# peterropac/Aegolius

Measured on AMD Instinct MI355X. Metric: Mpoints/sec SDF eval, 1024^3 grid, 10-prim smooth-union tree, higher is better.
Workload: dtype f32

## Files before the change

aegolius_amd/csrc/sdfk_codegen.cpp:

```cpp
#include "sdfk_codegen.h"

#include <algorithm>
#include <cstdio>
#include <cstring>
#include <map>
#include <set>

#include "sdfk_embedded.inc"

std::string sdfk_vector_prelude() { return std::string(kEmbeddedDevice) + "\n" + kEmbeddedVecdev + "\n"; }

static const char kWrappers[] = R"SDFKW(
template <int VEC, typename SRC>
static __device__ __forceinline__ void sdfk_body(const float* __restrict__ PRM, const float* __restrict__ TAB,
                                                 const SRC& src, long long off, long long n,
                                                 float* __restrict__ out, const float* __restrict__ aux,
                                                 long long aux_stride, unsigned* __restrict__ flags, unsigned thr) {
    const long long block_base = (long long)sdfk_bx() * (SDFK_BLOCK * VEC);
    const unsigned lane_off = sdfk_tx() * VEC;
#ifdef SDFK_FLAGS                                              // the flag-writing build of this flavour (its own code object:
    {                                                          // carried as a run-time branch it cost the field kernels registers)
        const bool active = block_base + lane_off < n;
        unsigned nib = 0u;
        if (active) {
// ... 737 lines not shown
        if (__builtin_bit_cast(unsigned, x0) != __builtin_bit_cast(unsigned, meta->xy[b][SDFK_RROWS - 1].x)) {
            int s = 1;
            while (s < SDFK_RROWS - 1 && __builtin_bit_cast(unsigned, meta->xy[b][s].x) == __builtin_bit_cast(unsigned, x0)) ++s;
            r0 = sb / NZP ? s : 0;
            r1 = sb / NZP ? SDFK_RROWS : s;
        }
    }
    const float2 pa = meta->xy[b][r0], pe = meta->xy[b][r1 - 1];
    const float za = meta->z[b][r0 * SDFK_RZ + i0], ze = meta->z[b][(r1 - 1) * SDFK_RZ + i0 + ZPS - 1];
    const float cx = 0.5f * (pa.x + pe.x), cy = 0.5f * (pa.y + pe.y), cz = 0.5f * (za + ze);
    float r2 = 0.0f;
#pragma unroll 1
    for (int rr = r0; rr < r1; ++rr) {
        const int r = rr - r0;
        const float2 p = meta->xy[b][r0 + r];
        const float dx = p.x - cx, dy = p.y - cy;
        float zm = 0.0f;
#pragma unroll
        for (int i = 0; i < ZPS; i += 4) {
            const float4 q = *reinterpret_cast<const float4*>(&meta->z[b][(r0 + r) * SDFK_RZ + i0 + i]);
            zm = sd_rawmax(sd_rawmax(zm, sd_abs(q.x - cz)), sd_rawmax(sd_abs(q.y - cz), sd_rawmax(sd_abs(q.z - cz), sd_abs(q.w - cz))));
        }
        r2 = sd_rawmax(r2, sd_fma(zm, zm, sd_fma(dx, dx, dy * dy)));
    }
    const float rho = 1.00001f * sqrtf(r2) + 1e-30f;
#ifdef SDFK_FLAT
    return make_float4(cx, cz, cy, rho);                         // (the staged coordinate is y, xy holds (x, z = 0))
#else
    return make_float4(cx, cy, cz, rho);
#endif
}
#endif

#if defined(SDFK_CHAIN) && !defined(SDFK_CELLS)
// Chain mode, one WAVE per brick: which children run on this brick, from the leaf values at its centre. A hard min (max:
// signs flipped, e_k = +-d_k) is exact, associative and commutative, so the ORDER of the chain does not matter for a
// decision: child k can be dropped wherever some other child j stays below it on the whole brick, and with j = the child
// that is smallest at the centre that is guaranteed by e_k - m >= thr, m = min_j e_j, thr = K rho + margins with
// K = the largest Lipschitz sum of the chain (any pair). No prefix minimum, no "restart" level: one reduction for m, then
// 64 children per step — compare, ballot, and the survivors written as a LIST in index order, so that the evaluation
// never looks at a child it skips and still combines the others in the chain's order. (Tighter than the sequential rule,
// which compares a child with its predecessors only.)
static __device__ __forceinline__ void sdfk_chain_fold(sdfk_rowmeta* meta, int b, int lane) {
    const float4 cc = meta->bound[b];
    const float rho = cc.w, cmag = 1e-6f * (fabsf(cc.x) + fabsf(cc.y) + fabsf(cc.z) + rho);
    constexpr int NW = (SDFK_NLEAF + 63) / 64;
    float m = 3.0e38f;
#pragma unroll 4
    for (int j = 0; j < NW; ++j) {
        const int k = 64 * j + lane;
        if (k < SDFK_NLEAF) m = fminf(m, SDFK_CHAIN_SGN * meta->leafval[k * SDFK_NCEN + b]);
    }
#pragma unroll
    for (int o = 1; o < 64; o <<= 1) m = fminf(m, __shfl_xor(m, o));
    const float thr0 = 1.0001f * SDFK_CHAIN_KMAX * rho + SDFK_CHAIN_KMAX * cmag + 1e-6f * (1.0f + fabsf(m));
    int n_out = 0;
#pragma unroll 1
    for (int j = 0; j < NW; ++j) {
        const int k = 64 * j + lane;
        const bool in = k < SDFK_NLEAF;
        const float e = in ? SDFK_CHAIN_SGN * meta->leafval[k * SDFK_NCEN + b] : 3.0e38f;
        const bool run = in && !(e - m >= thr0 + 1e-6f * fabsf(e));
        const unsigned long long bits = __ballot(run);
        if (run) meta->alist[b][n_out + __builtin_popcountll(bits & ((1ull << lane) - 1ull))] = (unsigned short)k;
        n_out += __builtin_popcountll(bits);
    }
    if (lane == 0) meta->nalive[b] = (unsigned)n_out;
}
#endif

#ifdef SDFK_CELLS
// rows of row block rb plus the cell of brick (rb, window c) and that cell's sphere (wave-uniform; scalar loads)
static __device__ __forceinline__ void sdfk_brick_cell(const sdfk_rowgeom& g, const sdfk_cells& cl, unsigned rb, unsigned c,
                                                       long long& r0, long long& rend, uint2& span, float4& S) {
    unsigned slot, blk;
    sdfk_block_rows(g, rb, r0, rend, &slot, &blk);
    const unsigned sx = slot == 0xffffffffu ? 0u : cl.lv.xoff + slot;
    const unsigned cell = ((sx >> cl.lv.lx) * cl.lv.ncy + (blk >> cl.lv.ly)) * cl.lv.ncz + (c >> cl.lv.lz);
    S = make_float4(0.0f, 0.0f, 0.0f, -1.0f);
    span = make_uint2(0u, SDFK_ALL_ALIVE);
    // (the launch is padded with bricks beyond the last one: their row block does not exist, and neither does a cell for it)
    if (cl.enabled && r0 < rend && cell < cl.ncells) {
        const uint2 sp = cl.span[cell];
        span = make_uint2(__builtin_amdgcn_readfirstlane(sp.x), __builtin_amdgcn_readfirstlane(sp.y));
        const float4 t = cl.sph[cell];
#ifdef SDFK_FLAT
        S = make_float4(t.x, t.z, t.y, t.w);                   // (the registers of phase A hold (x, z, y))
#else
        S = t;
#endif
    }
}
#endif
#if defined(SDFK_CHAIN) && defined(SDFK_CELLS)
// The same decision from the CELL's candidate list: one member per lane, evaluated at the brick's centre on the spot (no
// table of leaf values in LDS) — the first 64 stay in a register, longer lists are evaluated a second time for the
// comparison. A brick that is not inside its cell's sphere, or whose cell has no list, takes every member.
// `sp` (the cell's span) and `first` (this lane's entry of the first batch) were loaded BEFORE the coordinates were waited
// for, so the only memory round trip left between the bounds and the decision is the members' parameters.
static __device__ __forceinline__ void sdfk_chain_fold_cells(sdfk_rowmeta* meta, int b, int lane, const sdfk_cells& cl, uint2 sp,
                                                             unsigned first, const float* __restrict__ PRM,
                                                             const float* __restrict__ TAB) {
    const float4 cc = meta->bound[b];
    const V3T<float> ctr = {cc.x, cc.y, cc.z};
    const float rho = cc.w, cmag = 1e-6f * (fabsf(cc.x) + fabsf(cc.y) + fabsf(cc.z) + rho);
    unsigned off = 0u, cnt = SDFK_NLEAF;
    bool listed = false;
    if (cl.enabled && __builtin_amdgcn_readfirstlane(meta->inside[b]) != 0u && sp.y != SDFK_ALL_ALIVE) {
        off = sp.x; cnt = sp.y; listed = true;
    }
    float m = 3.0e38f, e0 = 3.0e38f;
    unsigned r0 = 0u;
#pragma unroll 1
    for (unsigned j0 = 0u; j0 < cnt; j0 += 64u) {
        const unsigned j = j0 + (unsigned)lane;
        const bool in = j < cnt;
        unsigned rec = 0u;
        if (in) rec = listed ? (j0 == 0u ? first : cl.cand[off + j]) : sdfk_member_record(j);
        float e = 3.0e38f;
        if (in) e = SDFK_CHAIN_SGN * sdfk_leaf_rec<float>(rec, ctr, PRM, TAB);
        if (j0 == 0u) { e0 = e; r0 = rec; }
        m = fminf(m, e);
    }
#pragma unroll
    for (int o = 1; o < 64; o <<= 1) m = fminf(m, __shfl_xor(m, o));
    const float thr0 = 1.0001f * SDFK_CHAIN_KMAX * rho + SDFK_CHAIN_KMAX * cmag + 1e-6f * (1.0f + fabsf(m));
    unsigned n_out = 0u;
#pragma unroll 1
    for (unsigned j0 = 0u; j0 < cnt; j0 += 64u) {
        const unsigned j = j0 + (unsigned)lane;
        const bool in = j < cnt;
        unsigned rec = r0;
        float e = e0;
        if (j0 != 0u) {
            rec = in ? (listed ? cl.cand[off + j] : sdfk_member_record(j)) : 0u;
            e = 3.0e38f;
            if (in) e = SDFK_CHAIN_SGN * sdfk_leaf_rec<float>(rec, ctr, PRM, TAB);
        }
        const bool run = in && !(e - m >= thr0 + 1e-6f * fabsf(e));
        const unsigned long long bits = __ballot(run);
        const unsigned pos = n_out + (unsigned)__builtin_popcountll(bits & ((1ull << lane) - 1ull));
        if (run && pos < SDFK_ALIST_CAP) meta->alist[b][pos] = rec;
        n_out += (unsigned)__builtin_popcountll(bits);
    }
    // more survivors than the list in LDS holds (dense scenes): the brick runs its cell's whole candidate list straight from
    // memory — a superset in the chain's order — and every member only where there is no such list
    if (lane == 0) {
        meta->nalive[b] = n_out <= SDFK_ALIST_CAP ? n_out : (listed ? SDFK_LIST_ALIVE : SDFK_ALL_ALIVE);
        meta->aspan[b] = make_uint2(off, cnt);
    }
}
#endif

// phases A and B of the tile of this workgroup; returns this wave's first brick (row block, window)
#ifdef SDFK_CELLS
#define SDFK_CELLS_PARAM , const sdfk_cells& cl
#define SDFK_CELLS_PASS , cl
#else
#define SDFK_CELLS_PARAM
#define SDFK_CELLS_PASS
#endif
template <typename SRC>
static __device__ __forceinline__ void sdfk_rows_prepare(const float* __restrict__ PRM, const float* __restrict__ TAB,
                                                         const SRC& s, const sdfk_rowgeom& g, sdfk_rowmeta* meta,
                                                         unsigned tile, unsigned& rb0, unsigned& c0 SDFK_CELLS_PARAM) {
    const int lane = sdfk_tx() & 63, wave = __builtin_amdgcn_readfirstlane(sdfk_tx() >> 6);
    const unsigned q0 = tile * SDFK_RNBRICK + wave * SDFK_RWBRICKS;            // first brick of this wave
    rb0 = sdfk_udiv(q0, g.nchunk, g.inv_nchunk);                // (back in an SGPR: what is derived from it stays scalar)
    c0 = q0 - rb0 * g.nchunk;
    unsigned rb = rb0, c = c0;
#if SDFK_RWBRICKS <= 2 && !defined(SDFK_NOHOIST)
    // two-wave workgroups on the north-star grid; with four bricks per wave the registers this takes cost more)
    sdfk_rowregs hregs[SDFK_RWBRICKS];
    bool live[SDFK_RWBRICKS];
#ifdef SDFK_CELLS
    uint2 cspan[SDFK_RWBRICKS];
    unsigned cfirst[SDFK_RWBRICKS];
    float4 csph[SDFK_RWBRICKS];
#endif
#pragma unroll
    for (int j = 0; j < SDFK_RWBRICKS; ++j) {
        long long r0, rend;
#ifdef SDFK_CELLS
        sdfk_brick_cell(g, cl, rb, c, r0, rend, cspan[j], csph[j]);
        cfirst[j] = 0u;                                          // the lane's entry of the list's first batch: in flight with the coordinates
        if (cspan[j].y != SDFK_ALL_ALIVE && (unsigned)lane < cspan[j].y) cfirst[j] = cl.cand[cspan[j].x + (unsigned)lane];
#else
        sdfk_block_rows(g, rb, r0, rend);
#endif
        live[j] = q0 + j < g.nbricks && r0 < rend;               // (blocks of the last plane beyond the slab: nothing)
        if (live[j]) sdfk_rows_load(s, g, r0, rend, c, lane, hregs[j]);
        if (++c == g.nchunk) { c = 0; ++rb; }
    }
#pragma unroll
    for (int j = 0; j < SDFK_RWBRICKS; ++j)
#ifdef SDFK_CELLS
        if (live[j]) sdfk_rows_bounds(hregs[j], lane, meta, wave * SDFK_RWBRICKS + j, csph[j]);
#else
        if (live[j]) sdfk_rows_bounds(hregs[j], lane, meta, wave * SDFK_RWBRICKS + j);
#endif
        else if (lane == 0) { meta->bound[wave * SDFK_RWBRICKS + j] = make_float4(0.0f, 0.0f, 0.0f, 1.0f); meta->uniform[wave * SDFK_RWBRICKS + j] = 0u; }   // (masks: never read)
#else
#ifdef SDFK_CELLS
    bool live[SDFK_RWBRICKS];
    uint2 cspan[SDFK_RWBRICKS];
    unsigned cfirst[SDFK_RWBRICKS];
#endif
#pragma unroll
    for (int j = 0; j < SDFK_RWBRICKS; ++j) {
        long long r0, rend;
#ifdef SDFK_CELLS
        float4 csph;
        sdfk_brick_cell(g, cl, rb, c, r0, rend, cspan[j], csph);
        cfirst[j] = 0u;
        if (cspan[j].y != SDFK_ALL_ALIVE && (unsigned)lane < cspan[j].y) cfirst[j] = cl.cand[cspan[j].x + (unsigned)lane];
        live[j] = q0 + j < g.nbricks && r0 < rend;
#else
        sdfk_block_rows(g, rb, r0, rend);
#endif
#ifdef SDFK_ABLATE_EDGE
        if (q0 + j < g.nbricks && r0 < rend && sdfk_interior(g.L, c)) {
#else
        if (q0 + j < g.nbricks && r0 < rend) {
#endif
            sdfk_rowregs regs;
            sdfk_rows_load(s, g, r0, rend, c, lane, regs);
#ifdef SDFK_CELLS
            sdfk_rows_bounds(regs, lane, meta, wave * SDFK_RWBRICKS + j, csph);
#else
            sdfk_rows_bounds(regs, lane, meta, wave * SDFK_RWBRICKS + j);
#endif
        } else if (lane == 0) {                                   // a dead brick still meets a probe lane: harmless values
            meta->bound[wave * SDFK_RWBRICKS + j] = make_float4(0.0f, 0.0f, 0.0f, 1.0f);
            meta->uniform[wave * SDFK_RWBRICKS + j] = 0u;
        }
        if (++c == g.nchunk) { c = 0; ++rb; }
    }
#endif
    __syncthreads();
#if defined(SDFK_CHAIN) && defined(SDFK_CELLS)
    // every wave folds ITS bricks from their cells' lists: nothing crosses waves any more (no probe centres, no table of
    // leaf values, two barriers fewer than the path below)
#pragma unroll
    for (int j = 0; j < SDFK_RWBRICKS; ++j) {
        const int b = wave * SDFK_RWBRICKS + j;
#ifdef SDFK_ABLATE_PROBE
        if (lane == 0) { meta->alist[b][0] = sdfk_member_record(0u); meta->nalive[b] = live[j] ? 1u : 0u; }
#else
        if (live[j]) sdfk_chain_fold_cells(meta, b, lane, cl, cspan[j], cfirst[j], PRM, TAB);
        else if (lane == 0) meta->nalive[b] = 0u;
#endif
    }
    __syncthreads();
    return;
#endif
#if defined(SDFK_SIMT) && !defined(SDFK_CELLS)
    // lane-parallel probe: probe centres -> every leaf at every centre (all lanes) -> one fold lane per centre ANDs its
    // skip decisions into the brick's mask (a subtree is skipped only if every sub-brick allows it)
    if (sdfk_tx() < SDFK_NCEN) {
        const unsigned b = sdfk_tx() / SDFK_NSUB, sb = sdfk_tx() % SDFK_NSUB;
        float4 cc = meta->bound[b];
#if SDFK_NSUB > 1
        if (meta->uniform[b]) cc = sdfk_sub_centre(meta, b, sb);
#else
        (void)sb;
#endif
        meta->cen[sdfk_tx()] = cc;
    }
    __syncthreads();
#ifndef SDFK_ABLATE_PROBE
    sdfk_probe_leaves(meta->cen, meta->leafval, PRM, TAB);
    __syncthreads();
#ifdef SDFK_CHAIN
#pragma unroll 1
    for (int j = 0; j < SDFK_RWBRICKS; ++j)
        if (q0 + j < g.nbricks) sdfk_chain_fold(meta, wave * SDFK_RWBRICKS + j, lane);
    __syncthreads();
    return;
#else
    if (sdfk_tx() < SDFK_NCEN && tile * SDFK_RNBRICK + sdfk_tx() / SDFK_NSUB < g.nbricks) {
        const float4 cc = meta->cen[sdfk_tx()];
        V3T<float> ctr = {cc.x, cc.y, cc.z};
        unsigned long long mk[SDFK_NMASK];
        sdfk_probe_fold(meta->leafval, sdfk_tx(), ctr, cc.w, PRM, mk);
#pragma unroll
        for (int w = 0; w < SDFK_NMASK; ++w)
            __hip_atomic_fetch_and(&meta->mask[w][sdfk_tx() / SDFK_NSUB], mk[w], __ATOMIC_RELAXED, __HIP_MEMORY_SCOPE_WORKGROUP);
    }
#endif
#else
    if (sdfk_tx() < SDFK_RNBRICK) {
#pragma unroll
        for (int w = 0; w < SDFK_NMASK; ++w) meta->mask[w][sdfk_tx()] = 0ull;
    }
#endif
    __syncthreads();
    return;
#endif
    if (sdfk_tx() < SDFK_RNBRICK && tile * SDFK_RNBRICK + sdfk_tx() < g.nbricks) {
        const float4 bb = meta->bound[sdfk_tx()];
        V3T<float> ctr = {bb.x, bb.y, bb.z};
        unsigned long long mk[SDFK_NMASK];
#pragma unroll
        for (int w = 0; w < SDFK_NMASK; ++w) mk[w] = 0ull;
#if !defined(SDFK_ABLATE_PROBE) && !defined(SDFK_CHAIN)
        sdfk_probe_r(ctr, bb.w, PRM, TAB, mk);
#endif
#pragma unroll
        for (int w = 0; w < SDFK_NMASK; ++w) meta->mask[w][sdfk_tx()] = mk[w];
    }
    __syncthreads();
}

template <typename SRC>
static __device__ __forceinline__ void sdfk_rows_kernel(const float* __restrict__ PRM, const float* __restrict__ TAB,
                                                        const SRC& s, const sdfk_rowgeom& g, float* __restrict__ out,
                                                        unsigned* __restrict__ flags, unsigned thr SDFK_CELLS_PARAM) {
    __shared__ __attribute__((aligned(16))) sdfk_rowmeta meta;
#ifdef SDFK_LDSPAD
    if (g.L == 0xffffffffu) meta.pad[sdfk_tx()] = 1.0f;
#endif
    const int lane = sdfk_tx() & 63, wave = __builtin_amdgcn_readfirstlane(sdfk_tx() >> 6);
    const int lr = lane / SDFK_RLPR;
    const int zq = (lane % SDFK_RLPR) * (2 * SDFK_NP);
#ifndef SDFK_RTILES
#define SDFK_RTILES 1
#endif
#ifndef SDFK_XGROUP
#ifdef SDFK_FLAT                         // flat grids (rows of 16385 points: 513 windows): short runs — the 50-member union at
#define SDFK_XGROUP 4
#else
#define SDFK_XGROUP (SDFK_RNBRICK <= 4 ? 16 : (SDFK_RNBRICK <= 8 ? 8 : 4))    // runs of about 64 bricks: two row blocks at 1025
#endif
#endif
#pragma unroll 1
  for (unsigned tt = 0; tt < SDFK_RTILES; ++tt) {
    // Workgroups go round-robin to the 8 XCDs: an XCD takes runs of SDFK_XGROUP consecutive tiles (the grid is a
    // multiple of 8 * SDFK_XGROUP) instead of every eighth tile, while all XCDs stay in the same neighbourhood of the
    // in all of them (DESIGN 9.1).
    const unsigned xg_t = sdfk_bx() / 8;
    const unsigned tile = (((xg_t / SDFK_XGROUP) * 8 + sdfk_bx() % 8) * SDFK_XGROUP + xg_t % SDFK_XGROUP) * SDFK_RTILES + tt;
    if (tile * SDFK_RNBRICK >= g.nbricks) break;
    if (tt) __syncthreads();
    unsigned rb, c;
    sdfk_rows_prepare(PRM, TAB, s, g, &meta, tile, rb, c SDFK_CELLS_PASS);
    const unsigned q0 = tile * SDFK_RNBRICK + wave * SDFK_RWBRICKS;
#pragma unroll 1
    for (int j = 0; j < SDFK_RWBRICKS; ++j) {
        if (q0 + j >= g.nbricks) break;
        const int b = wave * SDFK_RWBRICKS + j;
        const unsigned k = c;
        long long r0, rend;
        sdfk_block_rows(g, rb, r0, rend);
        if (++c == g.nchunk) { c = 0; ++rb; }
        if (r0 >= rend) continue;
        unsigned mw[2 * SDFK_NMASK];                             // the brick's skip bits as scalar words
#pragma unroll
        for (int w = 0; w < SDFK_NMASK; ++w) {
            const unsigned long long m = meta.mask[w][b];
            mw[2 * w] = __builtin_amdgcn_readfirstlane((unsigned)m);
            mw[2 * w + 1] = __builtin_amdgcn_readfirstlane((unsigned)(m >> 32));
        }
        const bool uniform = __builtin_amdgcn_readfirstlane(meta.uniform[b]) != 0u;
        const bool interior = sdfk_interior(g.L, k);
#ifdef SDFK_ABLATE_EDGE
        if (!interior) continue;
#endif
        const bool live_row = r0 + lr < rend;
        const int dr = live_row ? lr : (int)(rend - 1 - r0);
        long long f;                                              // flat index of this lane's first point
        const int z = sdfk_win_z(r0 + dr, g.L, k, zq, &f);        // its index in the row (edge chunks: may lie outside)
        const int last = (int)g.L - 1;
        V3P P[SDFK_NP];
        f2 res[SDFK_NP];
        // the staged coordinate: z (SDFK_FLAT: y, see sdfk_rows_load)
#ifdef SDFK_FLAT
        SDFK_EACH P[q].y = *reinterpret_cast<const f2*>(&meta.z[b][lr * SDFK_RZ + zq + 2 * q]);
#else
        SDFK_EACH P[q].z = *reinterpret_cast<const f2*>(&meta.z[b][lr * SDFK_RZ + zq + 2 * q]);
#endif
#ifdef SDFK_ABLATE_EVAL
        if (true) {
#ifdef SDFK_FLAT
            SDFK_EACH res[q] = P[q].y + __builtin_bit_cast(float, mw[0] ^ mw[1] ^ mw[2] ^ mw[3]);
#else
            SDFK_EACH res[q] = P[q].z + __builtin_bit_cast(float, mw[0] ^ mw[1] ^ mw[2] ^ mw[3]);
#endif
        } else
#endif
        if (uniform) {
            const float2 xy = meta.xy[b][lr];
#ifdef SDFK_FLAT
            SDFK_EACH { P[q].x = sp<f2>(xy.x); P[q].z = sp<f2>(xy.y); }      // (x, 0)
#else
            SDFK_EACH { P[q].x = sp<f2>(xy.x); P[q].y = sp<f2>(xy.y); }
#endif
#ifndef SDFK_CHAIN
            sdfk_rows_culled<true>(xy.x, xy.y, P, mw, PRM, TAB, res);
#endif
        } else {                                                  // the other coordinates of every point again (L2-resident)
#pragma unroll
            for (int q = 0; q < SDFK_NP; q += 2) {
                float4 X, Y, Z;
                sdfk_rows_fetch(s, g, r0, dr, z + 2 * q, interior, X, Y, Z);
                P[q].x = {X.x, X.y};
                P[q + 1].x = {X.z, X.w};
#ifdef SDFK_FLAT
                P[q].z = {Z.x, Z.y};
                P[q + 1].z = {Z.z, Z.w};
#else
                P[q].y = {Y.x, Y.y};
                P[q + 1].y = {Y.z, Y.w};
#endif
            }
#ifndef SDFK_CHAIN
            sdfk_rows_culled<false>(0.0f, 0.0f, P, mw, PRM, TAB, res);
#endif
        }
#ifdef SDFK_CHAIN
        {   // The children on the brick's list, in order; the first one starts the accumulator. Looked up one by one — kind of
            // the child, base of its parameters, then the parameters: three dependent scalar loads per child — the evaluation
            // the next SDFK_CHUNK children lane-parallel — a lane per (child, parameter) — into LDS, and then evaluates them
            // from there: the latency is paid once per chunk.
#ifdef SDFK_CELLS
            // (more survivors than the list holds — nalive = ALL —: every member, in order, straight from its index)
            const unsigned nal = __builtin_amdgcn_readfirstlane(meta.nalive[b]);
            const bool all_alive = nal == SDFK_ALL_ALIVE, list_alive = nal == SDFK_LIST_ALIVE;
            const unsigned aoff = __builtin_amdgcn_readfirstlane(meta.aspan[b].x);
            const unsigned cnt = all_alive ? (unsigned)SDFK_NLEAF : (list_alive ? __builtin_amdgcn_readfirstlane(meta.aspan[b].y) : nal);
#define SDFK_AREC(i) (all_alive ? sdfk_member_record(i) : (list_alive ? cl.cand[aoff + (i)] : meta.alist[b][i]))
#else
            const unsigned cnt = __builtin_amdgcn_readfirstlane(meta.nalive[b]);
#define SDFK_AREC(i) sdfk_member_record((unsigned)meta.alist[b][i])
#endif
            f2 acc[SDFK_NP];
#if SDFK_CHAIN_STAGED
            if (cnt <= SDFK_STAGE_MIN)
#endif
            {
                // one or two survivors (the 50-child flat union: 1.06 per brick): staging costs more than it hides, and
                // parameters in SGPRs beat parameters read back from LDS — straight from the table
#pragma unroll 1
                for (unsigned i = 0; i < cnt; ++i) {
                    const unsigned rec = __builtin_amdgcn_readfirstlane(SDFK_AREC(i));
                    f2 val[SDFK_NP];
                    SDFK_EACH val[q] = sdfk_leaf_rec<f2>(rec, P[q], PRM, TAB);
                    if (i == 0u) { SDFK_EACH acc[q] = val[q]; }
                    else { SDFK_EACH acc[q] = SDFK_CHAIN_CMB(acc[q], val[q], PRM); }
                }
            }
#if SDFK_CHAIN_STAGED
            else
#pragma unroll 1
            for (unsigned c0 = 0; c0 < cnt; c0 += SDFK_CHUNK) {
                const unsigned nc = cnt - c0 < SDFK_CHUNK ? cnt - c0 : SDFK_CHUNK;
                __builtin_amdgcn_fence(__ATOMIC_RELEASE, "wavefront");      // (the previous chunk has been read)
                __builtin_amdgcn_wave_barrier();
#pragma unroll 1
                for (unsigned it = (unsigned)lane; it < nc * SDFK_NPLMAX; it += 64u) {
                    const unsigned ch = it / SDFK_NPLMAX, w = it - ch * SDFK_NPLMAX;
                    const unsigned rec = SDFK_AREC(c0 + ch);
                    const unsigned at = (rec & 0xffffffu) + w;
                    meta.cprm[b][ch][w] = PRM[at < SDFK_NPARAMS ? at : SDFK_NPARAMS - 1u];
                    if (w == 0u) meta.cgrp[b][ch] = rec >> 24;
                }
                __builtin_amdgcn_fence(__ATOMIC_RELEASE, "wavefront");
                __builtin_amdgcn_wave_barrier();
                __builtin_amdgcn_fence(__ATOMIC_ACQUIRE, "wavefront");
#pragma unroll 1
                for (unsigned i = 0; i < nc; ++i) {
                    const unsigned grp = __builtin_amdgcn_readfirstlane(meta.cgrp[b][i]);
                    const float* cp = &meta.cprm[b][i][0];
                    f2 val[SDFK_NP];
                    SDFK_EACH val[q] = sdfk_leaf_at<f2>(grp, P[q], cp, TAB);
                    if (c0 + i == 0u) { SDFK_EACH acc[q] = val[q]; }
                    else { SDFK_EACH acc[q] = SDFK_CHAIN_CMB(acc[q], val[q], PRM); }
                }
            }
#endif
            SDFK_EACH res[q] = sdfk_chain_tail<f2>(acc[q], P[q], PRM, TAB);
#if defined(SDFK_DEBUG_NALIVE) && defined(SDFK_CELLS)
            // test aid: instead of the field, how the brick ran — survivors on its list; 100000 + entries when it ran its cell's
            // whole list (more survivors than SDFK_ALIST_CAP); -1 when it ran every member
            SDFK_EACH res[q] = sp<f2>(all_alive ? -1.0f : (list_alive ? 100000.0f + (float)cnt : (float)cnt));
#endif
        }
#endif
#ifdef SDFK_FLAGS                                                  // (the flag-writing build) one bit per point instead of the field
        {
            // BRICK-TILED layout: the word of (row r, window k) is flags[(brick * 16 + r % 16)], so the 64 lanes of the
            // wave — lane = 4 * row + octet of the window — write the brick's 64 bytes as ONE contiguous store, and every
            // (row, window) slot belongs to one brick, also where two rows share a flat window: no atomics (a linear bit
            // string needs an atomic OR in the edge windows and 16 partial-line stores per brick). The compaction
            unsigned bits = 0u;
            SDFK_EACH bits |= ((sdfk_sel_key(res[q].x) <= thr ? 1u : 0u) | (sdfk_sel_key(res[q].y) <= thr ? 2u : 0u)) << (2 * q);
            if (!interior) {                                       // an edge window: only the points of this row
                unsigned ok = 0u;
                SDFK_EACH {
                    if (z + 2 * q >= 0 && z + 2 * q <= last) ok |= 1u << (2 * q);
                    if (z + 2 * q + 1 >= 0 && z + 2 * q + 1 <= last) ok |= 2u << (2 * q);
                }
                bits &= ok;
            }
            if (!live_row) bits = 0u;                              // rows past the end of the last block: empty slots
            reinterpret_cast<unsigned char*>(flags)[(unsigned long long)(q0 + j) * 64ull + (unsigned)lane] = (unsigned char)bits;
        }
#else
        if (live_row) {
            float* po = out + f;
            if (interior) {
#pragma unroll
                for (int q = 0; q < SDFK_NP; q += 2) {
                    sdfk_f4u v = {res[q].x, res[q].y, res[q + 1].x, res[q + 1].y};
                    __builtin_nontemporal_store(v, reinterpret_cast<sdfk_f4u*>(po + 2 * q));
                }
            } else {
                SDFK_EACH {
                    if (z + 2 * q >= 0 && z + 2 * q <= last) po[2 * q] = res[q].x;
                    if (z + 2 * q + 1 >= 0 && z + 2 * q + 1 <= last) po[2 * q + 1] = res[q].y;
                }
            }
        }
#endif
    }
  }
}
#ifdef SDFK_WPE
#define SDFK_ROWS_ATTR __attribute__((amdgpu_waves_per_eu(SDFK_WPE, SDFK_WPE)))
#else
#define SDFK_ROWS_ATTR
#endif
#ifdef SDFK_CELLS
#define SDFK_CELLS_KARG , sdfk_cells cl
// ---- the pre-pass: one WAVE per cell ------------------------------------------------------------------------------
struct sdfk_cellpass {
    sdfk_celllevel lv, parent;                  // parent.ncx == 0: no coarser level — the candidates are all members
    float4* __restrict__ sph;                   // this level's cells: sphere ...
    uint2* __restrict__ span;                   // ... and list
    const float4* __restrict__ psph;            // the parent level's
    const uint2* __restrict__ pspan;
    unsigned* __restrict__ cand;                // the pool (records: sdfk_member_record)
    unsigned* __restrict__ head;                // this level's SDFK_POOL_SHARDS allocation heads, 64 bytes apart
    unsigned base, shard_cap;                   // shard h owns entries [base + h * shard_cap, base + (h + 1) * shard_cap)
    unsigned ncells, pad0;
    float inflate, pad;                         // factor on the radius the LIST is computed for (coarse level: > 1, see below)
};
// point z of local row `row`
static __device__ __forceinline__ float3 sdfk_cell_point(const SrcArray& s, const sdfk_rowgeom& g, long long row, unsigned z) {
    const float* p = s.co + row * (long long)g.L + z;
#ifdef SDFK_XY
    return make_float3(p[0], p[s.stride], 0.0f);
#else
    return make_float3(p[0], p[s.stride], p[2 * s.stride]);
#endif
}
static __device__ __forceinline__ float3 sdfk_cell_point(const SrcGrid& s, const sdfk_rowgeom& g, long long row, unsigned z) {
    const unsigned long long g0 = (unsigned long long)(g.row0 + row);
    if (g.yrows) return make_float3(s.ax0[g0], s.ax1[z], s.ax2[0]);
    const unsigned long long ix = g0 / s.n1;
    return make_float3(s.ax0[ix], s.ax1[(unsigned)(g0 - ix * s.n1)], s.ax2[z]);
}
// rows [r0, rend) and blocks of plane slot sl of a level (slot 0 = the leading partial plane when lv.xoff > 0)
static __device__ __forceinline__ bool sdfk_slot_rows(const sdfk_rowgeom& g, const sdfk_celllevel& lv, unsigned sl, long long& r0,
                                                      long long& rend) {
    if (lv.xoff > 0u && sl == 0u) { r0 = 0; rend = g.seg0; return g.seg0 > 0u; }
    if (sl < lv.xoff) return false;
    r0 = (long long)g.seg0 + (long long)(sl - lv.xoff) * g.prow;
    rend = r0 + g.prow < g.R ? r0 + g.prow : g.R;
    return r0 < g.R;
}
// ... 15 lines not shown
    if (sB == sA) { rb0 = ra0; rb1 = ra1; }
    const long long lo = (long long)(cy << lv.ly) * SDFK_RROWS, hi = (long long)((cy + 1u) << lv.ly) * SDFK_RROWS;
    some = some && ra0 + lo < ra1;
    const unsigned w0 = cz << lv.lz, w1 = ((cz + 1u) << lv.lz) < g.nchunk ? ((cz + 1u) << lv.lz) - 1u : g.nchunk - 1u;
    some = some && w0 < g.nchunk;
    if (!some) {                                                // no brick maps here
        if (lane == 0) { cp.sph[cell] = make_float4(0.0f, 0.0f, 0.0f, -1.0f); cp.span[cell] = make_uint2(0u, 0u); }
        return;
    }
    // windows are aligned in the FLAT array: window k of a row starts up to 31 points before point 32 k of that row
    const unsigned zlo = 32u * w0 > 31u ? 32u * w0 - 31u : 0u;
    const unsigned zhi = 32u * w1 + 31u < g.L ? 32u * w1 + 31u : g.L - 1u;
    // the eight corner points (a lattice cell is their convex hull): lanes 0..7
    const long long rowsel[4] = {ra0 + lo, (ra0 + hi < ra1 ? ra0 + hi : ra1) - 1, (rb0 + lo < rb1 ? rb0 + lo : rb1 - 1),
                                 (rb0 + hi < rb1 ? rb0 + hi : rb1) - 1};
    const float3 pt = sdfk_cell_point(s, g, rowsel[(lane >> 1) & 3], (lane & 1) ? zhi : zlo);
    float mnx = pt.x, mxx = pt.x, mny = pt.y, mxy = pt.y, mnz = pt.z, mxz = pt.z;
#pragma unroll
    for (int o = 1; o < 8; o <<= 1) {
        mnx = fminf(mnx, __shfl_xor(mnx, o)); mxx = fmaxf(mxx, __shfl_xor(mxx, o));
        mny = fminf(mny, __shfl_xor(mny, o)); mxy = fmaxf(mxy, __shfl_xor(mxy, o));
        mnz = fminf(mnz, __shfl_xor(mnz, o)); mxz = fmaxf(mxz, __shfl_xor(mxz, o));
    }
    const V3T<float> ctr = {0.5f * (mnx + mxx), 0.5f * (mny + mxy), 0.5f * (mnz + mxz)};
    const float dx = pt.x - ctr.x, dy = pt.y - ctr.y, dz = pt.z - ctr.z;
    float r2 = dx * dx + dy * dy + dz * dz;
#pragma unroll
    for (int o = 1; o < 8; o <<= 1) r2 = fmaxf(r2, __shfl_xor(r2, o));
    r2 = __shfl(r2, 0);
    const float cxs = __shfl(ctr.x, 0), cys = __shfl(ctr.y, 0), czs = __shfl(ctr.z, 0);
    const V3T<float> c = {cxs, cys, czs};
    // the radius the cell ANSWERS for: bricks test their points against it. A coarse level answers for more than its own
    // sphere (cp.inflate): the circumsphere of a fine cell can reach beyond the circumsphere of the coarse cell it lies in
    // (fine box at a corner, boxes of different proportions), and a fine cell may only start from its parent's list if its
    // whole sphere lies inside what that list answers for.
    const float rho = (1.0001f * sqrtf(r2) + 1e-30f) * cp.inflate;
    if (lane == 0) cp.sph[cell] = make_float4(c.x, c.y, c.z, rho);
    // candidates: the parent's list if this cell's sphere lies inside the parent's answer, else every member
    unsigned off = 0u, cnt = SDFK_NLEAF;
    bool listed = false;
    if (cp.parent.ncx != 0u) {
        unsigned pcx = 0u;
        if (!(lv.xoff > 0u && cx == 0u)) pcx = (cp.parent.xoff + (sA - lv.xoff)) >> cp.parent.lx;
        const unsigned pcell = (pcx * cp.parent.ncy + (cy >> (cp.parent.ly - lv.ly))) * cp.parent.ncz + (cz >> (cp.parent.lz - lv.lz));
        const float4 ps = cp.psph[pcell];
        const uint2 sp = cp.pspan[pcell];
        const float ex = c.x - ps.x, ey = c.y - ps.y, ez = c.z - ps.z;
        if (ps.w > 0.0f && sp.y != SDFK_ALL_ALIVE && 1.00002f * (sqrtf(ex * ex + ey * ey + ez * ez) + rho) <= ps.w) {
            off = sp.x; cnt = sp.y; listed = true;
        }
    }
    const float cmag = 1e-6f * (fabsf(c.x) + fabsf(c.y) + fabsf(c.z) + rho);
    // The candidates' values at the centre: the first SDFK_CELL_NB batches of 64 stay in registers (one evaluation per
    // candidate); what lies beyond is evaluated again for the count and once more for the write.
#ifndef SDFK_CELL_NB
#define SDFK_CELL_NB 8
#endif
#define SDFK_POOL_SHARDS 256u                   // (host: prepare_cells)
    float ev[SDFK_CELL_NB];
    unsigned rv[SDFK_CELL_NB];
    float m = 3.0e38f;
#pragma unroll
    for (int bt = 0; bt < SDFK_CELL_NB; ++bt) {
        const unsigned j = 64u * bt + (unsigned)lane;
        ev[bt] = 3.0e38f;
        rv[bt] = 0u;
        if (64u * bt < cnt) {
            if (j < cnt) {
                rv[bt] = listed ? cp.cand[off + j] : sdfk_member_record(j);
                ev[bt] = SDFK_CHAIN_SGN * sdfk_leaf_rec<float>(rv[bt], c, PRM, TAB);
            }
            m = fminf(m, ev[bt]);
        }
    }
#pragma unroll 4
    for (unsigned j0 = 64u * SDFK_CELL_NB; j0 < cnt; j0 += 64u) {
        const unsigned j = j0 + (unsigned)lane;
        if (j < cnt) m = fminf(m, SDFK_CHAIN_SGN * sdfk_leaf_rec<float>(listed ? cp.cand[off + j] : sdfk_member_record(j), c, PRM, TAB));
    }
#pragma unroll
    for (int o = 1; o < 64; o <<= 1) m = fminf(m, __shfl_xor(m, o));
    const float thr0 = 1.0001f * SDFK_CHAIN_KMAX * rho + SDFK_CHAIN_KMAX * cmag + 1e-6f * (1.0f + fabsf(m));
    unsigned total = 0u;
#pragma unroll
    for (int bt = 0; bt < SDFK_CELL_NB; ++bt)
        if (64u * bt < cnt) total += (unsigned)__builtin_popcountll(__ballot(64u * bt + (unsigned)lane < cnt && !(ev[bt] - m >= thr0 + 1e-6f * fabsf(ev[bt]))));
#pragma unroll 4
    for (unsigned j0 = 64u * SDFK_CELL_NB; j0 < cnt; j0 += 64u) {
        const unsigned j = j0 + (unsigned)lane;
        bool run = false;
        if (j < cnt) {
            const float e = SDFK_CHAIN_SGN * sdfk_leaf_rec<float>(listed ? cp.cand[off + j] : sdfk_member_record(j), c, PRM, TAB);
            run = !(e - m >= thr0 + 1e-6f * fabsf(e));
        }
        total += (unsigned)__builtin_popcountll(__ballot(run));
    }
    // per microsecond and address), so the pool is cut into SDFK_POOL_SHARDS shards with a head each, dealt by cell index
    unsigned at = 0u;
    const unsigned shard = cell & (SDFK_POOL_SHARDS - 1u);
    if (lane == 0) at = atomicAdd(cp.head + 16u * shard, total);
    at = __shfl(at, 0);
    if (at > cp.shard_cap || total > cp.shard_cap - at) {       // the shard is full: bricks of this cell probe every member
        if (lane == 0) cp.span[cell] = make_uint2(0u, SDFK_ALL_ALIVE);
        return;
    }
    at += cp.base + shard * cp.shard_cap;
    unsigned n_out = 0u;
#pragma unroll
    for (int bt = 0; bt < SDFK_CELL_NB; ++bt)
        if (64u * bt < cnt) {
            const bool run = 64u * bt + (unsigned)lane < cnt && !(ev[bt] - m >= thr0 + 1e-6f * fabsf(ev[bt]));
            const unsigned long long bits = __ballot(run);
            if (run) cp.cand[at + n_out + (unsigned)__builtin_popcountll(bits & ((1ull << lane) - 1ull))] = rv[bt];
            n_out += (unsigned)__builtin_popcountll(bits);
        }
#pragma unroll 4
    for (unsigned j0 = 64u * SDFK_CELL_NB; j0 < cnt; j0 += 64u) {
        const unsigned j = j0 + (unsigned)lane;
        bool run = false;
        unsigned rec = 0u;
        if (j < cnt) {
            rec = listed ? cp.cand[off + j] : sdfk_member_record(j);
            const float e = SDFK_CHAIN_SGN * sdfk_leaf_rec<float>(rec, c, PRM, TAB);
            run = !(e - m >= thr0 + 1e-6f * fabsf(e));
        }
        const unsigned long long bits = __ballot(run);
        if (run) cp.cand[at + n_out + (unsigned)__builtin_popcountll(bits & ((1ull << lane) - 1ull))] = rec;
        n_out += (unsigned)__builtin_popcountll(bits);
    }
    if (lane == 0) cp.span[cell] = make_uint2(at, total);
}
#else
#define SDFK_CELLS_KARG
#endif
)SDFKR";
static const char kRowsArray[] = R"SDFKR(
extern "C" __global__ __launch_bounds__(64 * SDFK_RWAVES) SDFK_ROWS_ATTR void sdfk_spec_r(
    const float* __restrict__ PRM, const float* __restrict__ TAB, const float* __restrict__ co, long long stride,
    sdfk_rowgeom g, float* __restrict__ out, unsigned* __restrict__ flags, unsigned thr SDFK_CELLS_KARG) {
    const SrcArray s = {co, stride};
    sdfk_rows_kernel(PRM, TAB, s, g, out, flags, thr SDFK_CELLS_PASS);
}
#ifdef SDFK_CELLS
extern "C" __global__ __launch_bounds__(256) void sdfk_spec_cells(
    const float* __restrict__ PRM, const float* __restrict__ TAB, const float* __restrict__ co, long long stride,
    sdfk_rowgeom g, sdfk_cellpass cp) {
    const SrcArray s = {co, stride};
    sdfk_cells_kernel(PRM, TAB, s, g, cp);
}
#endif
)SDFKR";
static const char kRowsGrid[] = R"SDFKR(
// the same on a regular grid expanded from three per-axis tables (no coordinate array: 4 B/point); the slab
// starts at a row boundary and out[0] is its first point
extern "C" __global__ __launch_bounds__(64 * SDFK_RWAVES) void sdfk_spec_rg(
    const float* __restrict__ PRM, const float* __restrict__ TAB, SrcGrid s, sdfk_rowgeom g, float* __restrict__ out,
    unsigned* __restrict__ flags, unsigned thr SDFK_CELLS_KARG) {
    sdfk_rows_kernel(PRM, TAB, s, g, out, flags, thr SDFK_CELLS_PASS);
}
#ifdef SDFK_CELLS
extern "C" __global__ __launch_bounds__(256) void sdfk_spec_cellsg(
    const float* __restrict__ PRM, const float* __restrict__ TAB, SrcGrid s, sdfk_rowgeom g, sdfk_cellpass cp) {
    sdfk_cells_kernel(PRM, TAB, s, g, cp);
}
#endif
)SDFKR";
static const char kRowsMask[] = R"SDFKR(
// test aid: the skip masks (two 64-bit words per brick: sites 0-31, 32-63; bit 2k = first operand of site k
// skipped, bit 2k+1 = second) followed by the "uniform rows" flag in a third word
extern "C" __global__ __launch_bounds__(64 * SDFK_RWAVES) void sdfk_spec_rmask(
    const float* __restrict__ PRM, const float* __restrict__ TAB, const float* __restrict__ co, long long stride,
    sdfk_rowgeom g, unsigned long long* __restrict__ masks) {
    __shared__ __attribute__((aligned(16))) sdfk_rowmeta meta;
    const SrcArray s = {co, stride};
    unsigned rb, c;
    sdfk_rows_prepare(PRM, TAB, s, g, &meta, sdfk_bx(), rb, c);
    const unsigned q = sdfk_bx() * SDFK_RNBRICK + sdfk_tx();
    if (sdfk_tx() < SDFK_RNBRICK && q < g.nbricks) {
        masks[3ull * q] = meta.mask[0][sdfk_tx()];
        masks[3ull * q + 1] = meta.mask[1][sdfk_tx()];
        masks[3ull * q + 2] = meta.uniform[sdfk_tx()];
    }
}
)SDFKR";

namespace {

struct Gen {
    const sdfk_opinfo* ops;
    int n_ops;
    const uint32_t* code;
    size_t n_instr;
    const std::vector<sdfk_cullsite>* sites;
    std::string s;
    bool rows = false;

    std::vector<int> root_slot;
    int n_root = 0;
    void find_roots() {
        root_slot.assign(n_instr, -1);
        bool c0_intact = true;
        for (size_t i = 0; i < n_instr; ++i) {
            const uint32_t w = code[2 * i];
            const unsigned op = w & 255u, a = (w >> 8) & 255u, b = (w >> 16) & 255u;
            if ((int)op >= n_ops) continue;
            if (ops[op].kind != SDFK_KIND_C_C) continue;
            if (!strcmp(ops[op].name, "XFORM") && b == 0 && c0_intact && n_root < 64) root_slot[i] = n_root++;
            if (a == 0) c0_intact = false;
        }
    }

    void instr_x(size_t i, const char* indent, int mode) {
        const int r = root_slot.empty() ? -1 : root_slot[i];
        if (r < 0 || mode == 0 || (rows && mode == 1)) {
            instr(i, indent, rows && mode == 2);
            return;
        }
        char buf[1400];
        const uint32_t w = code[2 * i], poff = code[2 * i + 1];
        const unsigned a = (w >> 8) & 255u;
        if (rows) {
            snprintf(buf, sizeof buf,
                     "%sif constexpr (ZRUN) {\n"
                     "#ifdef SDFK_FLAT\n"
                     "%s  const V3T<float> bs = op_xform_base_x(X, PRM + %u);\n"
                     "%s  const V3P bp = {sp<f2>(bs.x), sp<f2>(bs.y), sp<f2>(bs.z)};\n"
                     "%s  SDFK_EACH C_%u[q] = op_xform_y(bp, C_0[q].y, PRM + %u);\n"
                     "#else\n"
                     "%s  const V3T<float> bs = op_xform_base(X, Y, PRM + %u);\n"
                     "%s  const V3P bp = {sp<f2>(bs.x), sp<f2>(bs.y), sp<f2>(bs.z)};\n"
                     "%s  SDFK_EACH C_%u[q] = op_xform_z(bp, C_0[q].z, PRM + %u);\n"
                     "#endif\n"
                     "%s} else { SDFK_EACH C_%u[q] = op_xform(C_0[q], PRM + %u, TAB, 0); }\n",
                     indent, indent, poff, indent, indent, a, poff, indent, poff, indent, indent, a, poff, indent, a, poff);
        } else if (mode == 1) {
            snprintf(buf, sizeof buf,
                     "%s{ const V3T<float> bs = op_xform_base(C_0.x, C_0.y, PRM + %u); bases[%d] = bs.x; bases[%d] = bs.y; "
                     "bases[%d] = bs.z;\n%s  C_%u = op_xform_z(bs, C_0.z, PRM + %u); }\n",
                     indent, poff, 3 * r, 3 * r + 1, 3 * r + 2, indent, a, poff);
        } else {
            snprintf(buf, sizeof buf,
                     "%sif constexpr (ZRUN) { const V3T<T> bs = {sp<T>(bases[%d]), sp<T>(bases[%d]), sp<T>(bases[%d])};\n"
                     "%s  C_%u = op_xform_z(bs, C_0.z, PRM + %u); }\n%selse C_%u = op_xform(C_0, PRM + %u, TAB, 0);\n",
                     indent, 3 * r, 3 * r + 1, 3 * r + 2, indent, a, poff, indent, a, poff);
        }
        s += buf;
    }

    void instr(size_t i, const char* indent) { instr(i, indent, false); }
    void instr(size_t i, const char* indent, bool arr) {
        char buf[256];
        const uint32_t w = code[2 * i], poff = code[2 * i + 1];
        const unsigned op = w & 255u, a = (w >> 8) & 255u, b = (w >> 16) & 255u, c = w >> 24;
        if ((int)op >= n_ops) return;
        const sdfk_opinfo& o = ops[op];
        if (!strcmp(o.name, "V_FIELD")) {
            snprintf(buf, sizeof buf, "%sV_%u = sdfk_aux<T>(AUX, AUXS, %u);\n", indent, a, c);
            s += buf;
            return;
        }
        const char* e = arr ? "SDFK_EACH " : "";
        const char* x = arr ? "[q]" : "";
        switch (o.kind) {
            case SDFK_KIND_C_C:
                snprintf(buf, sizeof buf, "%s%sC_%u%s = %s(C_%u%s, PRM + %u, TAB, %u);\n", indent, e, a, x, o.func, b, x, poff, c);
                break;
            case SDFK_KIND_V_C:
                snprintf(buf, sizeof buf, "%s%sV_%u%s = %s(C_%u%s, PRM + %u, TAB);\n", indent, e, a, x, o.func, b, x, poff);
                break;
            case SDFK_KIND_V_V:
                snprintf(buf, sizeof buf, "%s%sV_%u%s = %s(V_%u%s, PRM + %u);\n", indent, e, a, x, o.func, b, x, poff);
                break;
            default:
                snprintf(buf, sizeof buf, "%s%sV_%u%s = %s(V_%u%s, V_%u%s, PRM + %u);\n", indent, e, a, x, o.func, b, x, c, x, poff);
                break;
        }
        s += buf;
    }

    void declare(const char* ctype, const char* vtype, bool arr, bool init = false) {
        std::set<unsigned> cregs, vregs;
        for (size_t i = 0; i < n_instr; ++i) {
            const uint32_t w = code[2 * i];
            const unsigned op = w & 255u, a = (w >> 8) & 255u;
            if ((int)op >= n_ops) continue;
            if (ops[op].kind == SDFK_KIND_C_C) cregs.insert(a);
            else vregs.insert(a);
        }
        char buf[160];
        const char* dim = arr ? "[SDFK_NP]" : "";
        const char* ini = init ? " = {}" : "";
        for (unsigned c : cregs)
            if (c != 0) {
                snprintf(buf, sizeof buf, "    %s C_%u%s;\n", ctype, c, dim);
                s += buf;
            }
        for (unsigned v : vregs) {
            snprintf(buf, sizeof buf, "    %s V_%u%s%s;\n", vtype, v, dim, ini);
            s += buf;
        }
    }

    int site_opening_at(size_t i, size_t hi) const {
        int best = -1;
        for (size_t k = 0; k < sites->size(); ++k) {
            const sdfk_cullsite& t = (*sites)[k];
            if (t.a0 == i && t.comb <= hi && (best < 0 || t.comb > (*sites)[best].comb)) best = (int)k;
// ... 876 lines not shown
```

Before: 366,900.

## Read grid coordinates directly from axis tables, skipping LDS staging

Adds a grid-specific path for the row kernel. Each lane reads x, y and eight z values straight from the per-axis tables, and the probe spheres are built from those registers with lane shuffles. This replaces the LDS staging of z, the row heads, the uniform flag and the 64-bit division. The x/y part of the root transforms is also done once per lane (rows_culled<true>). The cost is extra global/cached table reads and shuffle reductions per brick, and this path does not apply to chain mode or flat grids.

```diff
diff --git a/aegolius_amd/csrc/sdfk_codegen.cpp b/aegolius_amd/csrc/sdfk_codegen.cpp
--- a/aegolius_amd/csrc/sdfk_codegen.cpp
+++ b/aegolius_amd/csrc/sdfk_codegen.cpp
@@ -913,6 +913,231 @@
 }
 #endif
 
+// ---- grid flavour: coordinates straight from the axis tables -------------------------------------------------------
+// On a grid (SrcGrid) a row has one x and one y by construction and its z values are entries of ax2, so nothing has to
+// be loaded, staged or proven: a lane reads the coordinates of its own 8 points from the tables — lane = 4 * row + octet
+// of the window, in the probe exactly as in phase C — and the probe spheres come from the same registers with a few
+// lane exchanges. No LDS copy of z, no row heads, no "uniform" flag, no 64-bit division. Everything else — bricks,
+// windows, the tile enumeration, the probe, the fold, the masks, the stores — is the code the array build runs.
+// Selected by the source type (sdfk_direct<SRC>); -DSDFK_GRID_STAGED brings the staged skeleton back for the grid too.
+// Chain mode and flat grids always use the staged skeleton.
+template <typename SRC> struct sdfk_direct { static constexpr bool value = false; };
+template <typename SRC> struct sdfk_meta_of { typedef sdfk_rowmeta type; };
+static __device__ __forceinline__ bool sdfk_meta_uniform(const sdfk_rowmeta& meta, int b) {
+    return __builtin_amdgcn_readfirstlane(meta.uniform[b]) != 0u;
+}
+#if !defined(SDFK_GRID_STAGED) && !defined(SDFK_CHAIN) && !defined(SDFK_FLAT)
+static_assert(SDFK_NP == 4 && SDFK_RLPR == 4 && SDFK_RROWS == 16, "a lane owns 8 points: two 16-byte reads of ax2");
+struct sdfk_gridmeta {
+    float4 bound[SDFK_RNBRICK];                 // the brick's sphere (builds without the lane-parallel probe)
+    unsigned long long mask[SDFK_NMASK][SDFK_RNBRICK];
+#ifdef SDFK_SIMT
+    float4 cen[SDFK_NCEN];
+    float leafval[SDFK_NLEAF * SDFK_NCEN];
+#endif
+#ifdef SDFK_LDSPAD
+    float pad[SDFK_LDSPAD / 4];
+#endif
+};
+template <> struct sdfk_direct<SrcGrid> { static constexpr bool value = true; };
+template <> struct sdfk_meta_of<SrcGrid> { typedef sdfk_gridmeta type; };
+static __device__ __forceinline__ bool sdfk_meta_uniform(const sdfk_gridmeta&, int) { return true; }
+
+// first row of a block -> (plane, row of the plane): one wave-uniform 32-bit division per brick (multiply-high with the
+// reciprocal, as the compiler expands it) wherever the row index fits 32 bits; the 64-bit one is left for grids beyond
+// 2^32 rows
+static __device__ __forceinline__ void sdfk_grid_block(const SrcGrid& s, const sdfk_rowgeom& g, long long r0, unsigned long long& ix0,
+                                                       unsigned& iy0) {
+    const unsigned long long g0 = (unsigned long long)(g.row0 + r0);
+    if ((g0 >> 32) == 0ull) {
+        const unsigned q = (unsigned)g0 / s.n1;
+        ix0 = q;
+        iy0 = (unsigned)g0 - q * s.n1;
+    } else {
+        ix0 = g0 / s.n1;
+        iy0 = (unsigned)(g0 - ix0 * s.n1);
+    }
+}
+// The 8 points [z, z + 8) of local row r0 + dr (r0 wave-uniform, dr per lane): x, y and two quads of z.
+// Index safety. Callers pass only bricks that exist (q < g.nbricks) with r0 < rend, and dr in [0, rend - 1 - r0]: the
+// padded tiles and dead bricks of a launch never get here, and rows past the end of a partial last block have been
+// replaced by the block's last live row before dr is formed. So the global row G = g.row0 + r0 + dr lies in
+// [row0, row0 + R), and the host accepts a slab only if start + count <= n0 * n1 * n2 (row0 = start / n2, R = count / n2):
+// G < n0 * n1, hence ix < n0 and iy < n1, whatever row0, seg0 and nb0 are (a slab that starts mid-plane only makes iy0
+// non-zero). z comes from sdfk_win_z: in an interior window all 32 points lie in the row (sdfk_interior), so [z, z + 8) is
+// inside [0, L); in the two edge windows of a row (L no multiple of 32) every index is clamped to [0, L - 1], L = n2.
+// (ix, iy0): plane and row of the plane of local row r0 (sdfk_grid_block).
+static __device__ __forceinline__ void sdfk_grid_fetch(const SrcGrid& s, const sdfk_rowgeom& g, unsigned long long ix, unsigned iy0,
+                                                       int dr, int z, bool interior, float& x, float& y, float4& Za, float4& Zb) {
+    // the lane's own row: carries into the next planes (one at most unless a plane has fewer than 16 rows)
+    const unsigned room = s.n1 - iy0;                             // rows left in plane ix, at least one
+    unsigned t = (unsigned)dr;
+    if (t >= room) {
+        t -= room;
+        ++ix;
+        while (t >= s.n1) { t -= s.n1; ++ix; }
+    } else {
+        t += iy0;
+    }
+    x = s.ax0[ix];
+    y = s.ax1[t];
+    if (interior) {
+        const sdfk_f4u a = *reinterpret_cast<const sdfk_f4u*>(s.ax2 + z), b = *reinterpret_cast<const sdfk_f4u*>(s.ax2 + z + 4);
+        Za = make_float4(a.x, a.y, a.z, a.w);
+        Zb = make_float4(b.x, b.y, b.z, b.w);
+    } else {
+        const int last = (int)g.L - 1;
+        Za = make_float4(s.ax2[min(max(z, 0), last)], s.ax2[min(max(z + 1, 0), last)], s.ax2[min(max(z + 2, 0), last)],
+                         s.ax2[min(max(z + 3, 0), last)]);
+        Zb = make_float4(s.ax2[min(max(z + 4, 0), last)], s.ax2[min(max(z + 5, 0), last)], s.ax2[min(max(z + 6, 0), last)],
+                         s.ax2[min(max(z + 7, 0), last)]);
+    }
+}
+// Probe spheres of one live brick (wave-uniform r0, rend, k; the whole wave), NS of them to dst[0 .. NS): the sub-brick
+// layout of sdfk_sub_centre — 4 parts along the window x NS / 4 along the rows; NS = 1: the whole brick. Every lane holds
+// the 8 points phase C will give it; centre = midpoint of the sub-brick's first and last point, radius = the exact
+// maximum over its points, all taken from the table entries themselves (any table is bounded correctly: unequal steps,
+// descending, repeated, unordered). With two parts along the rows, a block that runs into the next plane is split where
+// the plane changes instead of in the middle (as the staged skeleton does where x changes); rows of further planes
+// (n1 < 16) stay in the second part, whose maximum runs over all of them.
+template <int NS>
+static __device__ __forceinline__ void sdfk_grid_spheres(const SrcGrid& s, const sdfk_rowgeom& g, long long r0, long long rend,
+                                                         unsigned k, int lane, float4* dst) {
+    constexpr int NZP = NS > 1 ? 4 : 1, NRP = NS / NZP, RPS = SDFK_RROWS / NRP, LPZ = SDFK_RLPR / NZP;
+    const int lr = lane / SDFK_RLPR, oc = lane % SDFK_RLPR;
+    const int nlive = rend - r0 < (long long)SDFK_RROWS ? (int)(rend - r0) : SDFK_RROWS;
+    const int dr = lr < nlive ? lr : nlive - 1;                   // rows past the end: the last live row again
+    long long f;
+    const int z = sdfk_win_z(r0 + dr, g.L, k, 8 * oc, &f);
+    unsigned long long ix0;
+    unsigned iy0;
+    sdfk_grid_block(s, g, r0, ix0, iy0);
+    float x, y;
+    float4 Za, Zb;
+    sdfk_grid_fetch(s, g, ix0, iy0, dr, z, sdfk_interior(g.L, k), x, y, Za, Zb);
+    int gr = lr / RPS, ra = gr * RPS, re = ra + RPS - 1;          // the lane's part along the rows: its first and last row
+    if constexpr (NRP == 2) {
+        const unsigned room = s.n1 - iy0;                         // rows of the block before the next plane
+        if (room < (unsigned)nlive) {
+            gr = (unsigned)lr >= room ? 1 : 0;
+            ra = gr ? (int)room : 0;
+            re = gr ? SDFK_RROWS - 1 : (int)room - 1;
+        }
+    }
+    const int zp = oc / LPZ;
+    const int la = ra * SDFK_RLPR + zp * LPZ, le = re * SDFK_RLPR + zp * LPZ + LPZ - 1;   // lanes of the first and last point
+    const float cx = 0.5f * (__shfl(x, la) + __shfl(x, le)), cy = 0.5f * (__shfl(y, la) + __shfl(y, le));
+    const float cz = 0.5f * (__shfl(Za.x, la) + __shfl(Zb.w, le));
+    const float dx = x - cx, dy = y - cy;
+    const float zm = sd_rawmax(sd_rawmax(sd_rawmax(sd_abs(Za.x - cz), sd_abs(Za.y - cz)), sd_rawmax(sd_abs(Za.z - cz), sd_abs(Za.w - cz))),
+                               sd_rawmax(sd_rawmax(sd_abs(Zb.x - cz), sd_abs(Zb.y - cz)), sd_rawmax(sd_abs(Zb.z - cz), sd_abs(Zb.w - cz))));
+    const float d2 = sd_fma(zm, zm, sd_fma(dx, dx, dy * dy));
+    float r2 = 0.0f;
+#pragma unroll
+    for (int p = 0; p < NRP; ++p) {                               // maximum over the lanes of part p (same part of the window)
+        float v = gr == p ? d2 : 0.0f;
+#pragma unroll
+        for (int o = 1; o < 64; o <<= 1)
+            if (o < LPZ || o >= SDFK_RLPR) v = sd_rawmax(v, __shfl_xor(v, o));
+        if (gr == p) r2 = v;
+    }
+    // written by a lane that is in part lr / RPS wherever the split falls: row 0 for the first part, the last row of the others
+    const int wp = lr / RPS;
+    if (oc % LPZ == 0 && lr == (wp == 0 ? 0 : wp * RPS + RPS - 1))
+        dst[wp * NZP + zp] = make_float4(cx, cy, cz, 1.00001f * sqrtf(r2) + 1e-30f);
+}
+// phases A and B of a tile, grid flavour: no loads, no staging; returns this wave's first brick like sdfk_rows_prepare
+static __device__ __forceinline__ void sdfk_grid_prepare(const float* __restrict__ PRM, const float* __restrict__ TAB,
+                                                         const SrcGrid& s, const sdfk_rowgeom& g, sdfk_gridmeta* meta,
+                                                         unsigned tile, unsigned& rb0, unsigned& c0) {
+    const int lane = sdfk_tx() & 63, wave = __builtin_amdgcn_readfirstlane(sdfk_tx() >> 6);
+    const unsigned q0 = tile * SDFK_RNBRICK + wave * SDFK_RWBRICKS;            // first brick of this wave
+    rb0 = sdfk_udiv(q0, g.nchunk, g.inv_nchunk);
+    c0 = q0 - rb0 * g.nchunk;
+    unsigned rb = rb0, c = c0;
+#ifdef SDFK_SIMT
+    constexpr int NS = SDFK_NSUB;
+#else
+    constexpr int NS = 1;
+#endif
+#pragma unroll
+    for (int j = 0; j < SDFK_RWBRICKS; ++j) {
+        const int b = wave * SDFK_RWBRICKS + j;
+#ifdef SDFK_SIMT
+        float4* dst = &meta->cen[b * NS];
+#else
+        float4* dst = &meta->bound[b];
+#endif
+        long long r0, rend;
+        sdfk_block_rows(g, rb, r0, rend);
+        // (dead bricks of a padded tile and blocks of the last plane beyond the slab: they still meet a probe lane — harmless
+        //  values, and no table is indexed for them)
+        if (q0 + j < g.nbricks && r0 < rend) sdfk_grid_spheres<NS>(s, g, r0, rend, c, lane, dst);
+        else if (lane < NS) dst[lane] = make_float4(0.0f, 0.0f, 0.0f, 1.0f);
+#ifdef SDFK_SIMT
+        if (lane < SDFK_NMASK) meta->mask[lane][b] = ~0ull;        // the fold lanes AND their decisions into these
+#endif
+        if (++c == g.nchunk) { c = 0; ++rb; }
+    }
+    __syncthreads();
+#ifdef SDFK_SIMT
+#ifndef SDFK_ABLATE_PROBE
+    sdfk_probe_leaves(meta->cen, meta->leafval, PRM, TAB);
+    __syncthreads();
+    if (sdfk_tx() < SDFK_NCEN && tile * SDFK_RNBRICK + sdfk_tx() / SDFK_NSUB < g.nbricks) {
+        const float4 cc = meta->cen[sdfk_tx()];
+        V3T<float> ctr = {cc.x, cc.y, cc.z};
+        unsigned long long mk[SDFK_NMASK];
+        sdfk_probe_fold(meta->leafval, sdfk_tx(), ctr, cc.w, PRM, mk);
+#pragma unroll
+        for (int w = 0; w < SDFK_NMASK; ++w)
+            __hip_atomic_fetch_and(&meta->mask[w][sdfk_tx() / SDFK_NSUB], mk[w], __ATOMIC_RELAXED, __HIP_MEMORY_SCOPE_WORKGROUP);
+    }
+#else
+    if (sdfk_tx() < SDFK_RNBRICK) {
+#pragma unroll
+        for (int w = 0; w < SDFK_NMASK; ++w) meta->mask[w][sdfk_tx()] = 0ull;
+    }
+#endif
+#else
+    if (sdfk_tx() < SDFK_RNBRICK && tile * SDFK_RNBRICK + sdfk_tx() < g.nbricks) {
+        const float4 bb = meta->bound[sdfk_tx()];
+        V3T<float> ctr = {bb.x, bb.y, bb.z};
+        unsigned long long mk[SDFK_NMASK];
+#pragma unroll
+        for (int w = 0; w < SDFK_NMASK; ++w) mk[w] = 0ull;
+#ifndef SDFK_ABLATE_PROBE
+        sdfk_probe_r(ctr, bb.w, PRM, TAB, mk);
+#endif
+#pragma unroll
+        for (int w = 0; w < SDFK_NMASK; ++w) meta->mask[w][sdfk_tx()] = mk[w];
+    }
+#endif
+    __syncthreads();
+}
+// phase C, grid flavour: the lane's 8 points from the tables, the x/y part of the root transforms once per lane
+static __device__ __forceinline__ void sdfk_grid_eval(const float* __restrict__ PRM, const float* __restrict__ TAB, const SrcGrid& s,
+                                                      const sdfk_rowgeom& g, long long r0, int dr, int z, bool interior,
+                                                      const unsigned (&mw)[2 * SDFK_NMASK], V3P (&P)[SDFK_NP], f2 (&res)[SDFK_NP]) {
+    unsigned long long ix0;
+    unsigned iy0;
+    sdfk_grid_block(s, g, r0, ix0, iy0);
+    float x, y;
+    float4 Za, Zb;
+    sdfk_grid_fetch(s, g, ix0, iy0, dr, z, interior, x, y, Za, Zb);
+    SDFK_EACH { P[q].x = sp<f2>(x); P[q].y = sp<f2>(y); }
+    P[0].z = {Za.x, Za.y};
+    P[1].z = {Za.z, Za.w};
+    P[2].z = {Zb.x, Zb.y};
+    P[3].z = {Zb.z, Zb.w};
+#ifdef SDFK_ABLATE_EVAL
+    SDFK_EACH res[q] = P[q].z + __builtin_bit_cast(float, mw[0] ^ mw[1] ^ mw[2] ^ mw[3]);
+#else
+    sdfk_rows_culled<true>(x, y, P, mw, PRM, TAB, res);
+#endif
+}
+#endif
+
 // phases A and B of the tile of this workgroup; returns this wave's first brick (row block, window)
 #ifdef SDFK_CELLS
 #define SDFK_CELLS_PARAM , const sdfk_cells& cl
@@ -1077,7 +1302,7 @@
 static __device__ __forceinline__ void sdfk_rows_kernel(const float* __restrict__ PRM, const float* __restrict__ TAB,
                                                         const SRC& s, const sdfk_rowgeom& g, float* __restrict__ out,
                                                         unsigned* __restrict__ flags, unsigned thr SDFK_CELLS_PARAM) {
-    __shared__ __attribute__((aligned(16))) sdfk_rowmeta meta;
+    __shared__ __attribute__((aligned(16))) typename sdfk_meta_of<SRC>::type meta;
 #ifdef SDFK_LDSPAD
     if (g.L == 0xffffffffu) meta.pad[sdfk_tx()] = 1.0f;
 #endif
@@ -1104,7 +1329,8 @@
     if (tile * SDFK_RNBRICK >= g.nbricks) break;
     if (tt) __syncthreads();
     unsigned rb, c;
-    sdfk_rows_prepare(PRM, TAB, s, g, &meta, tile, rb, c SDFK_CELLS_PASS);
+    if constexpr (sdfk_direct<SRC>::value) sdfk_grid_prepare(PRM, TAB, s, g, &meta, tile, rb, c);
+    else sdfk_rows_prepare(PRM, TAB, s, g, &meta, tile, rb, c SDFK_CELLS_PASS);
     const unsigned q0 = tile * SDFK_RNBRICK + wave * SDFK_RWBRICKS;
 #pragma unroll 1
     for (int j = 0; j < SDFK_RWBRICKS; ++j) {
@@ -1122,7 +1348,7 @@
             mw[2 * w] = __builtin_amdgcn_readfirstlane((unsigned)m);
             mw[2 * w + 1] = __builtin_amdgcn_readfirstlane((unsigned)(m >> 32));
         }
-        const bool uniform = __builtin_amdgcn_readfirstlane(meta.uniform[b]) != 0u;
+        const bool uniform = sdfk_meta_uniform(meta, b);
         const bool interior = sdfk_interior(g.L, k);
 #ifdef SDFK_ABLATE_EDGE
         if (!interior) continue;
@@ -1134,6 +1360,9 @@
         const int last = (int)g.L - 1;
         V3P P[SDFK_NP];
         f2 res[SDFK_NP];
+        if constexpr (sdfk_direct<SRC>::value) {
+            sdfk_grid_eval(PRM, TAB, s, g, r0, dr, z, interior, mw, P, res);
+        } else {   // the staged skeleton (arrays, chain mode, flat grids): the statements it always had, left where they were
         // the staged coordinate: z (SDFK_FLAT: y, see sdfk_rows_load)
 #ifdef SDFK_FLAT
         SDFK_EACH P[q].y = *reinterpret_cast<const f2*>(&meta.z[b][lr * SDFK_RZ + zq + 2 * q]);
@@ -1177,6 +1406,7 @@
 #ifndef SDFK_CHAIN
             sdfk_rows_culled<false>(0.0f, 0.0f, P, mw, PRM, TAB, res);
 #endif
+        }
         }
 #ifdef SDFK_CHAIN
         {   // The children on the brick's list, in order; the first one starts the accumulator. Looked up one by one — kind of
@@ -1498,7 +1728,8 @@
 )SDFKR";
 static const char kRowsGrid[] = R"SDFKR(
 // the same on a regular grid expanded from three per-axis tables (no coordinate array: 4 B/point); the slab
-// starts at a row boundary and out[0] is its first point
+// starts at a row boundary and out[0] is its first point. Phases A to C read the tables themselves (sdfk_grid_prepare,
+// sdfk_grid_eval) except in chain mode, on flat grids and under -DSDFK_GRID_STAGED, which run the array kernel's skeleton
 extern "C" __global__ __launch_bounds__(64 * SDFK_RWAVES) void sdfk_spec_rg(
     const float* __restrict__ PRM, const float* __restrict__ TAB, SrcGrid s, sdfk_rowgeom g, float* __restrict__ out,
     unsigned* __restrict__ flags, unsigned thr SDFK_CELLS_KARG) {
```

After: 366,700. About the same (-0.1%).
